# itailang/SampleNet

Hardware: NVIDIA H100
Metric: point-clouds/sec SampleNet fwd+Chamfer (B=32, N=1024->64) (higher is better)
Workload: dtype f32

## Files before the change

samplenet_b200/csrc/conv_stack.cu:

```cuda
#include "encoder_internal.cuh"
#include <cooperative_groups.h>
#include <string.h>

namespace snb {

constexpr int kCsMaxLayers = SNB200_MAX_CONV_LAYERS;
constexpr int kCsMaxSlicesPerCta = 32;
constexpr int kCsThreads = 512;
constexpr int kCsMaxPts = 128;
constexpr int kCsMinPts = 64;
constexpr int kCsNPT = kCsMaxPts / 4;
constexpr int kCsChunks = 4;
constexpr int kCsMaxSeg = 8;
constexpr int kCsLoPlane = kCsMaxPts * 128;
constexpr uint32_t kCsSlotBytes = 2u * kCsLoPlane;
constexpr int kCsWLd = 132;
constexpr uint32_t kCsWOff = kCsChunks * kCsSlotBytes;
constexpr uint32_t kCsAccOff = 2 * kCsSlotBytes;
constexpr size_t kCsSmemBytes = (size_t)kCsWOff + 128 * kCsWLd * sizeof(float) + 1024;

struct CsLayer {
    int c_in, c_out;
    const float *weight, *bias;
    const float *gamma, *beta, *run_mean, *run_var;
    float eps;
    int has_bn, relu;
    double *stats;
    float *zsave;
    int keep;
};

struct CsParams {
    const float *x; int layout;
    int b, n;
    long long total;
    int ppc, npt;
    int slots_per_cloud;
    int num_layers;
    CsLayer L[kCsMaxLayers];
    int training;
    double *mom;
    unsigned *barrier;
    float *tile_max, *tile_min;
    int fuse_head;
    HeadParams H;
    int self_clean;
    char *clean_ptr;
    unsigned clean_bytes;
    int slices_per_cta, num_slices;
    float *act[2];
    int act_ld;
    int head_rows;
};

__device__ __forceinline__ void cs_grid_arrive(unsigned *counter)
{
    asm volatile("red.release.gpu.global.add.u32 [%0], 1;" ::"l"(counter) : "memory");
}
__device__ __forceinline__ void cs_grid_wait(unsigned *counter, unsigned target)
{
    unsigned v, spin = 0;
    do {
        asm volatile("ld.acquire.gpu.global.u32 %0, [%1];" : "=r"(v) : "l"(counter) : "memory");
        if (++spin > (1u << 26)) __trap();
    } while (v < target);
}
__device__ __forceinline__ void cs_grid_barrier(unsigned *counter, unsigned target)
{
    __syncthreads();
    if (threadIdx.x == 0) {
        __threadfence();
        atomicAdd(counter, 1u);
        unsigned v, spin = 0;
        do {
            asm volatile("ld.acquire.gpu.global.u32 %0, [%1];" : "=r"(v) : "l"(counter) : "memory");
            if (++spin > (1u << 26)) __trap();
        } while (v < target);
    }
    __syncthreads();
}

__device__ __forceinline__ void cs_xchg_store(float *p, float v)
{
    unsigned u = __float_as_uint(v);
    if (u == 0u) u = 0x80000000u;
    asm volatile("st.volatile.global.u32 [%0], %1;" ::"l"(p), "r"(u) : "memory");
}
__device__ __forceinline__ unsigned cs_xchg_load1(const float *p)
{
    unsigned v;
    asm volatile("ld.volatile.global.u32 %0, [%1];" : "=r"(v) : "l"(p) : "memory");
    return v;
}
__device__ __forceinline__ uint4 cs_xchg_load4(const float *p)
{
    uint4 v;
    asm volatile("ld.volatile.global.v4.u32 {%0, %1, %2, %3}, [%4];" : "=r"(v.x), "=r"(v.y), "=r"(v.z), "=r"(v.w) : "l"(p) : "memory");
    return v;
}

__device__ __forceinline__ void cs_head_stage_weights(const HeadLayer &L, int cb, int nch, float *s_wh, int tid)
{
    const int c_in = L.c_in;
    if ((c_in & 3) == 0) {
        const int q4 = c_in >> 2, total = 8 * q4;
        for (int e0 = tid; e0 < total; e0 += kCsThreads * 4) {
            float4 v[4];
#pragma unroll
            for (int u = 0; u < 4; u++) {
                const int e = e0 + u * kCsThreads;
                const int jr = e / q4, kq = e - jr * q4;
                v[u] = (e < total && jr < nch) ? __ldg(reinterpret_cast<const float4 *>(L.weight + (size_t)(cb + jr) * c_in) + kq) : make_float4(0, 0, 0, 0);
// ... 90 lines not shown
    return v;
}
__device__ __forceinline__ void cs_named_sync(int id, int nthreads) { asm volatile("bar.sync %0, %1;" ::"r"(id), "r"(nthreads) : "memory"); }

#ifdef SNB200_CS_TIMELINE
constexpr int kCsTlMaxCtas = 256, kCsTlMaxSlices = 8;
constexpr int kCsTlPerLayer = 2 + 5 * kCsTlMaxSlices;
constexpr int kCsTlHead = 2 + (kCsMaxLayers - 1) * kCsTlPerLayer, kCsTlStamps = kCsTlHead + 2;
__device__ unsigned long long g_cs_tl[kCsTlMaxCtas][kCsTlStamps][2];
__device__ __forceinline__ int cs_tl_layer(int l) { return 2 + (l - 1) * kCsTlPerLayer; }
__device__ __forceinline__ void cs_tl_stamp(int idx)
{
    if (threadIdx.x == 0 && blockIdx.x < kCsTlMaxCtas && idx >= 0 && idx < kCsTlStamps) {
        unsigned long long c, t;
        asm volatile("mov.u64 %0, %%clock64;" : "=l"(c) :: "memory");
        asm volatile("mov.u64 %0, %%globaltimer;" : "=l"(t) :: "memory");
        g_cs_tl[blockIdx.x][idx][0] = c;
        g_cs_tl[blockIdx.x][idx][1] = t;
    }
}
#define CS_TL(idx) cs_tl_stamp(idx)
#define CS_TL_SLICE(l, t, k) do { if ((t) < kCsTlMaxSlices) cs_tl_stamp(cs_tl_layer(l) + 1 + 5 * (t) + (k)); } while (0)
#else
#define CS_TL(idx) do { } while (0)
#define CS_TL_SLICE(l, t, k) do { } while (0)
#endif

__device__ __forceinline__ void cs_copy_w(float *sW, const CsLayer &L, int ch, int g, uint64_t *bar)
{
    const int K = L.c_in, N = L.c_out;
    if (ch < N) {
        if (g == 0) {
            fence_proxy_async();
            if (ch == 0) mbar_expect_tx(bar, (uint32_t)(N * K) * 4u);
            tma_load_1d(sW + (size_t)ch * kCsWLd, L.weight + (size_t)ch * K, (uint32_t)K * 4u, bar);
        }
    } else {
        float4 *z = reinterpret_cast<float4 *>(sW + (size_t)ch * kCsWLd + g * (K >> 2));
#pragma unroll
        for (int i = 0; i < 8; i++)
            if (i * 16 < K) z[i] = make_float4(0.f, 0.f, 0.f, 0.f);
    }
}
__device__ __forceinline__ void cs_wait_w(uint64_t *bar, int c) { mbar_wait(bar, (uint32_t)c & 1u); }

__device__ __forceinline__ void cs_wg_wait_1() { asm volatile("wgmma.wait_group.sync.aligned 1;" ::: "memory"); }

__device__ __forceinline__ void cs_write_chunk(const uint32_t (&v)[kCsNPT], float sc, float sh, float floor_v, int npt, uint32_t base, uint32_t gsw)
{
#pragma unroll
    for (int jb = 0; jb < kCsNPT / 8; jb++) {
        if (jb * 8 < npt) {
#pragma unroll
            for (int i = 0; i < 8; i++) {
                const float t = fmaxf(fmaf(__uint_as_float(v[jb * 8 + i]), sc, sh), floor_v);
                const float h = tf32_hi(t);
                const uint32_t a = base + (gsw ^ (uint32_t)(i << 4)) + (uint32_t)(jb * 1024 + i * 128);
                asm volatile("st.shared.f32 [%0], %1;" ::"r"(a), "f"(h) : "memory");
                asm volatile("st.shared.f32 [%0], %1;" ::"r"(a + (uint32_t)kCsLoPlane), "f"(t - h) : "memory");
            }
        }
    }
}

__device__ __forceinline__ int cs_acc_idx(int pt, int ch) { return pt * 128 + (ch ^ (((pt >> 1) & 3) << 3)); }

__device__ __forceinline__ void cs_save_rows(float *dst, int ld, const uint32_t (&v)[kCsNPT], int nvalid)
{
#pragma unroll
    for (int j = 0; j < kCsNPT; j++)
        if (j < nvalid) dst[j * ld] = __uint_as_float(v[j]);
}

__device__ __forceinline__ void cs_load_rows(const float *src, int ld, uint32_t (&v)[kCsNPT], int nvalid)
{
#pragma unroll
    for (int j = 0; j < kCsNPT; j++) v[j] = (j < nvalid) ? __float_as_uint(__ldcg(src + j * ld)) : 0u;
}

template <bool kMulti>
__global__ void __launch_bounds__(kCsThreads, 1) conv_stack_kernel(const __grid_constant__ CsParams P)
{
    extern __shared__ __align__(1024) unsigned char smem_raw[];
    __shared__ __align__(16) float sX[kCsMaxPts * 3];
    __shared__ float sW1[128 * 3], sB1[128];
    __shared__ float sRedS[4][128], sRedQ[4][128];
    __shared__ double sMom[9];
    __shared__ float sMomW[kCsThreads / 32][9];
    __shared__ int sBad;
    __shared__ uint64_t sWbar;

    const int tid = threadIdx.x, warp = tid >> 5, lane = tid & 31;
    const int q = warp & 3, g = (warp >> 2) & 3;
    const int ch = q * 32 + lane;
    const int G = gridDim.x;
    const int ppc = P.ppc, npt = P.npt, n = P.n;
    const long long P0 = (long long)blockIdx.x * ppc;
    const int npts = (int)min((long long)ppc, P.total - P0);
    const int col0 = g * npt;
    const int nvalid = max(0, min(npt, npts - col0));
    unsigned char *smem = smem_raw + ((1024u - (smem_u32(smem_raw) & 1023u)) & 1023u);
    float *sW = reinterpret_cast<float *>(smem + kCsWOff);
    float *sAcc = reinterpret_cast<float *>(smem + kCsAccOff);
    CS_TL(0);

    if (tid < 9) sMom[tid] = 0.0;
    if (tid == 0) sBad = 0;
    if (warp == 1) {
        if (lane == 0) mbar_init(&sWbar, 1);
        fence_mbar_init();
    }
    const CsLayer &L1 = P.L[0];
    const int nslices = kMulti ? (P.num_slices - (int)blockIdx.x + G - 1) / G : 1;
    auto load_x_slice = [&](const long long P0s, const int nptss) {
        if (P.layout == SNB200_BNC) {
            const float *src = P.x + P0s * 3;
            const int nf = nptss * 3;
            for (int e = tid; e < ppc * 3; e += kCsThreads) sX[e] = (e < nf) ? __ldg(src + e) : 0.f;
        } else {
            for (int e = tid; e < ppc * 3; e += kCsThreads) {
                const int c = e / ppc, r = e - c * ppc;
                float xv = 0.f;
                if (r < nptss) {
                    const int gp = (int)P0s + r;
                    const int cloud = gp / n, pi = gp - cloud * n;
                    xv = __ldg(P.x + ((size_t)cloud * 3 + c) * n + pi);
                }
                sX[r * 3 + c] = xv;
            }
        }
    };
    if (!kMulti) load_x_slice(P0, npts);
    for (int e = tid; e < L1.c_out * 3; e += kCsThreads) sW1[e] = __ldg(L1.weight + e);
    for (int e = tid; e < L1.c_out; e += kCsThreads) sB1[e] = L1.bias ? __ldg(L1.bias + e) : 0.f;
    __syncthreads();
    unsigned barrier_epoch = 0;
    const bool need_stats = P.training != 0;
    if (P.self_clean) {
        float4 *z = reinterpret_cast<float4 *>(P.clean_ptr);
        const unsigned n16 = P.clean_bytes >> 4;
        for (unsigned e = blockIdx.x * kCsThreads + tid; e < n16; e += G * kCsThreads) z[e] = make_float4(0.f, 0.f, 0.f, 0.f);
        if (!(need_stats && L1.has_bn)) cs_grid_barrier(P.barrier, ++barrier_epoch * G);
    }

    cs_copy_w(sW, P.L[1], ch, g, &sWbar);

    if (need_stats && L1.has_bn) {
        const int mom_pts = kMulti ? ppc : npts;
        float a9[9] = {0, 0, 0, 0, 0, 0, 0, 0, 0};
        for (int t = 0; t < nslices; t++) {
            int nptss = npts;
            if (kMulti) {
                const long long P0s = (long long)((int)blockIdx.x + t * G) * ppc;
                nptss = (int)min((long long)ppc, P.total - P0s);
                __syncthreads();
                load_x_slice(P0s, nptss);
                __syncthreads();
            }
            if (tid < nptss) {
                const float px = sX[tid * 3 + 0], py = sX[tid * 3 + 1], pz = sX[tid * 3 + 2];
                a9[0] += px; a9[1] += py; a9[2] += pz;
                a9[3] = fmaf(px, px, a9[3]); a9[4] = fmaf(px, py, a9[4]); a9[5] = fmaf(px, pz, a9[5]);
                a9[6] = fmaf(py, py, a9[6]); a9[7] = fmaf(py, pz, a9[7]); a9[8] = fmaf(pz, pz, a9[8]);
            }
        }
        if (warp * 32 < mom_pts) {
#pragma unroll
            for (int j = 0; j < 9; j++) {
                float v = a9[j];
                for (int o = 16; o > 0; o >>= 1) v += __shfl_xor_sync(kFullMask, v, o);
                if (lane == 0) sMomW[warp][j] = v;
            }
        }
        __syncthreads();
        if (tid < 9) {
            double t = 0.0;
            for (int w = 0; w * 32 < mom_pts && w < kCsThreads / 32; w++) t += (double)sMomW[w][tid];
            atomicAdd(P.mom + tid, t);
            cs_grid_arrive(reinterpret_cast<unsigned *>(P.mom + 9));
        }
    }
    if (need_stats && L1.has_bn) {
        if (tid < 9) {
            cs_grid_wait(reinterpret_cast<unsigned *>(P.mom + 9), 9u * G);
            sMom[tid] = __ldcg(P.mom + tid);
        }
        __syncthreads();
    }
    CS_TL(1);

    uint32_t v[kCsNPT];
    auto layer1_eval = [&](const long long P0s, const int nvalids) {
        if (q * 32 < L1.c_out) {
            const bool cv = ch < L1.c_out;
            const float w0 = cv ? sW1[ch * 3 + 0] : 0.f, w1 = cv ? sW1[ch * 3 + 1] : 0.f, w2 = cv ? sW1[ch * 3 + 2] : 0.f, b1 = cv ? sB1[ch] : 0.f;
#pragma unroll
            for (int jb = 0; jb < kCsNPT / 8; jb++) {
                if (jb * 8 < npt) {
                    const float4 *xq = reinterpret_cast<const float4 *>(sX + (col0 + jb * 8) * 3);
                    float xr[24];
#pragma unroll
                    for (int u = 0; u < 6; u++) { const float4 t4 = xq[u]; xr[u * 4 + 0] = t4.x; xr[u * 4 + 1] = t4.y; xr[u * 4 + 2] = t4.z; xr[u * 4 + 3] = t4.w; }
#pragma unroll
                    for (int i = 0; i < 8; i++) v[jb * 8 + i] = __float_as_uint(fmaf(w2, xr[i * 3 + 2], fmaf(w1, xr[i * 3 + 1], w0 * xr[i * 3 + 0])) + b1);
                }
            }
            if (L1.zsave && cv) cs_save_rows(L1.zsave + ((int)P0s + col0) * L1.c_out + ch, L1.c_out, v, nvalids);
        }
    };
    if (!kMulti) layer1_eval(P0, nvalid);

    for (int l = 1; l < P.num_layers; l++) {
        const CsLayer &Lp = P.L[l - 1];
        const CsLayer &Lc = P.L[l];
        const int K = Lc.c_in, N = Lc.c_out;
        const int nchunks = K >> 5;
        const bool last = (l == P.num_layers - 1);
        const bool want_stats = need_stats && Lc.has_bn;

        {
            float sc = 1.f, sh = 0.f;
            if (Lp.has_bn && ch < K && g == 0) {
                const float pgamma = cs_ld_now(Lp.gamma + ch), pbeta = cs_ld_now(Lp.beta + ch);

                float mean, var;
                if (P.training) {
                    const double cnt = (double)P.total, inv_cnt = 1.0 / cnt;
                    double m, vv;
                    if (l == 1) {
                        const double mx = sMom[0] * inv_cnt, my = sMom[1] * inv_cnt, mz = sMom[2] * inv_cnt;
                        const double cxx = sMom[3] * inv_cnt - mx * mx, cxy = sMom[4] * inv_cnt - mx * my, cxz = sMom[5] * inv_cnt - mx * mz;
                        const double cyy = sMom[6] * inv_cnt - my * my, cyz = sMom[7] * inv_cnt - my * mz, czz = sMom[8] * inv_cnt - mz * mz;
                        const double a0 = sW1[ch * 3 + 0], a1 = sW1[ch * 3 + 1], a2 = sW1[ch * 3 + 2];
                        m = a0 * mx + a1 * my + a2 * mz + (double)sB1[ch];
                        vv = a0 * a0 * cxx + a1 * a1 * cyy + a2 * a2 * czz + 2.0 * (a0 * a1 * cxy + a0 * a2 * cxz + a1 * a2 * cyz);
                        if (vv < 0) vv = 0;
                        if (blockIdx.x == 0) {
                            Lp.stats[ch] = cnt * m;
                            Lp.stats[K + ch] = cnt * (vv + m * m);
                        }
                    } else {
                        double s1, s2;
                        cs_fx_collect(Lp.stats, K, ch, (unsigned)G, s1, s2);
                        if (blockIdx.x == 0) { Lp.stats[ch] = s1; Lp.stats[K + ch] = s2; }
                        m = s1 * inv_cnt;
                        vv = s2 * inv_cnt - m * m;
                        if (vv < 0) vv = 0;
                    }
                    mean = (float)m; var = (float)vv;
                } else {
                    mean = Lp.run_mean[ch]; var = Lp.run_var[ch];
                }
                const float invstd = 1.0f / sqrtf(var + Lp.eps);
                sc = pgamma * invstd;
                sh = pbeta - mean * sc;
            }
            if (Lp.has_bn) {
                if (g == 0 && ch < K) { sRedS[0][ch] = sc; sRedQ[0][ch] = sh; }
                cs_named_sync(1, kCsThreads);
                if (ch < K) { sc = sRedS[0][ch]; sh = sRedQ[0][ch]; }
                cs_named_sync(1, kCsThreads);
            }
            CS_TL(cs_tl_layer(l));
            const int mh = g & 1, nh = g >> 1;
            const bool mma_wg = mh * 64 < N && nh * 64 < ppc;
            const float bias = (ch < N && Lc.bias) ? __ldg(Lc.bias + ch) : 0.f;
            float sumL = 0.f, sqL = 0.f;
            const float *act_in = kMulti && l > 1 ? (Lp.zsave ? Lp.zsave : P.act[(l - 1) & 1]) : nullptr;
            float *act_out = kMulti && !last ? (Lc.zsave ? Lc.zsave : P.act[l & 1]) : Lc.zsave;
            const int ld_in = (kMulti && !Lp.zsave && P.act_ld) ? P.act_ld : K, ld_out = (kMulti && !last && !Lc.zsave && P.act_ld) ? P.act_ld : N;
            auto write_tiles = [&](const int sl, const int cl_first, const int nseg, const float *sPmax, const float *sPmin) {
                const int S = P.slots_per_cloud;
                for (int e = tid; e < nseg * N; e += kCsThreads) {
                    const int s = e / N, c = e - s * N;
                    const int cl = cl_first + s;
                    const int slot = sl - cl * n / ppc;
                    float mx = -INFINITY, mn = INFINITY;
#pragma unroll
                    for (int gg = 0; gg < 4; gg++) {
                        mx = fmaxf(mx, sPmax[(gg * kCsMaxSeg + s) * 128 + c]);
                        mn = fminf(mn, sPmin[(gg * kCsMaxSeg + s) * 128 + c]);
                    }
                    if (sBad) { mx = INFINITY; mn = -INFINITY; }
                    P.tile_max[((size_t)cl * S + slot) * N + c] = mx;
                    P.tile_min[((size_t)cl * S + slot) * N + c] = mn;
                    if (((cl + 1) * n - 1) / ppc == sl)
                        for (int s2 = slot + 1; s2 < S; s2++) {
                            P.tile_max[((size_t)cl * S + s2) * N + c] = -INFINITY;
                            P.tile_min[((size_t)cl * S + s2) * N + c] = INFINITY;
                        }
                }
            };
            int cl_first = 0, nseg = 0;
            float *sPmax = reinterpret_cast<float *>(smem);
            float *sPmin = sPmax + 4 * kCsMaxSeg * 128;
            for (int t = 0; t < nslices; t++) {
                const int tv = kMulti && (l & 1) ? nslices - 1 - t : t;
                const int sl = kMulti ? (int)blockIdx.x + tv * cs_nctaid() : (int)blockIdx.x;
                const long long P0 = (long long)sl * ppc;
                const int npts = (int)min((long long)ppc, P.total - P0);
                const int nvalid = max(0, min(npt, npts - col0));
                const bool lastslice = !kMulti || t == nslices - 1;
                const bool kept = kMulti && nslices - 1 - t < Lc.keep;
                if (kMulti) {
#pragma unroll
                    for (int j = 0; j < kCsNPT; j++) v[j] = 0u;
                    const bool on_chip = t < Lp.keep;
                    if (l == 1) {
                        if (!on_chip) {
                            __syncthreads();
                            load_x_slice(P0, npts);
                            __syncthreads();
                        }
                        layer1_eval(P0, nvalid);
                    } else if (on_chip && t == 0) {
                        const float pbias = (ch < K && Lp.bias) ? __ldg(Lp.bias + ch) : 0.f;
#pragma unroll
                        for (int j = 0; j < kCsNPT; j++) v[j] = __float_as_uint(sAcc[col0 * 128 + cs_acc_idx(j, ch)] + pbias);
                        if (nchunks > 2) __syncthreads();
                    } else if (ch < K) {
                        if (on_chip) {
                            const float *src = sW + col0 * kCsWLd + 64 + ch;
#pragma unroll
                            for (int j = 0; j < kCsNPT; j++) v[j] = (j < nvalid) ? __float_as_uint(src[j * kCsWLd]) : 0u;
                        } else {
                            cs_load_rows(act_in + ((int)P0 + col0) * ld_in + ch, ld_in, v, nvalid);
                        }
                    }
                }
                CS_TL_SLICE(l, t, 0);
                if (q < nchunks) {
                    const uint32_t base = smem_u32(smem) + (uint32_t)q * kCsSlotBytes + (uint32_t)col0 * 128u + (uint32_t)((lane & 3) << 2);
                    cs_write_chunk(v, sc, sh, Lp.relu ? 0.f : -INFINITY, npt, base, (uint32_t)((lane >> 2) << 4));
                    fence_proxy_async();
                }
                if (kMulti && lastslice && t > 0 && Lc.keep >= 2 && ch < N) {
#pragma unroll
                    for (int j = 0; j < kCsNPT; j++) v[j] = __float_as_uint(sAcc[col0 * 128 + cs_acc_idx(j, ch)] + bias);
                    cs_save_rows(sW + col0 * kCsWLd + 64 + ch, kCsWLd, v, npt);
                }
                if (t == 0 && tid == 0) cs_wait_w(&sWbar, l - 1);
                __syncthreads();
                CS_TL_SLICE(l, t, 1);
                float acc[32];
                if (mma_wg) {
#pragma unroll
                    for (int i = 0; i < 32; i++) acc[i] = 0.f;
                    const float *wrow = sW + (size_t)(mh * 64 + q * 16 + (lane >> 2)) * kCsWLd + (lane & 3);
                    const uint32_t bbase = smem_u32(smem) + (uint32_t)nh * 64u * 128u;
                    uint32_t ahi[2][4], alo[2][4];
#pragma unroll 1
                    for (int c = 0; c < nchunks; c++) {
                        const uint32_t sb = bbase + (uint32_t)c * kCsSlotBytes;
#pragma unroll
                        for (int ks = 0; ks < 4; ks++) {
                            float w[4];
#pragma unroll
                            for (int e = 0; e < 4; e++) w[e] = wrow[(e & 1) * 8 * kCsWLd + c * 32 + ks * 8 + (e >> 1) * 4];
                            cs_wg_wait_1();
#pragma unroll
                            for (int e = 0; e < 4; e++) {
                                const float h = tf32_hi(w[e]);
                                ahi[ks & 1][e] = __float_as_uint(h);
                                alo[ks & 1][e] = __float_as_uint(w[e] - h);
                            }
                            wg_fence();
                            const uint64_t b_hi = wg_sdesc(sb + (uint32_t)(ks * 32));
                            const uint64_t b_lo = wg_sdesc(sb + (uint32_t)(kCsLoPlane + ks * 32));
                            wg_mma_rs_n64(acc, alo[ks & 1], b_hi, (c > 0 || ks > 0) ? 1u : 0u);
                            wg_mma_rs_n64(acc, ahi[ks & 1], b_lo, 1u);
                            wg_mma_rs_n64(acc, ahi[ks & 1], b_hi, 1u);
                            wg_commit();
                        }
                    }
                    wg_wait_all();
                }
                CS_TL_SLICE(l, t, 2);
                __syncthreads();
                if (mma_wg) {
                    const int r0 = mh * 64 + q * 16 + (lane >> 2), cq = nh * 64 + 2 * (lane & 3);
                    float *st0 = sAcc + cs_acc_idx(cq, r0), *st8 = sAcc + cs_acc_idx(cq, r0 + 8);
#pragma unroll
                    for (int j = 0; j < 8; j++) {
                        st0[j * 1024] = acc[4 * j + 0];
                        st0[j * 1024 + 128] = acc[4 * j + 1];
                        st8[j * 1024] = acc[4 * j + 2];
                        st8[j * 1024 + 128] = acc[4 * j + 3];
                    }
                }
                __syncthreads();
                if (!last && lastslice) cs_copy_w(sW, P.L[l + 1], ch, g, &sWbar);
                cl_first = (int)P0 / n;
                nseg = ((int)P0 + npts - 1) / n - cl_first + 1;
#pragma unroll
                for (int j = 0; j < kCsNPT; j++) v[j] = __float_as_uint(sAcc[col0 * 128 + cs_acc_idx(j, ch)]);
                CS_TL_SLICE(l, t, 3);
                if (q * 32 < N) {
                    float sum = 0.f, sq = 0.f;
#pragma unroll
                    for (int j = 0; j < kCsNPT; j++) {
                        const float u = __uint_as_float(v[j]) + bias;
                        v[j] = __float_as_uint(u);
                        if (j < nvalid) { sum += u; sq = fmaf(u, u, sq); }
                    }
                    if (kMulti) { sumL += sum; sqL += sq; }
                    else if (want_stats) { sRedS[g][ch] = sum; sRedQ[g][ch] = sq; }
                    if (act_out && ch < N && (Lc.zsave || !kept)) cs_save_rows(act_out + ((int)P0 + col0) * ld_out + ch, ld_out, v, nvalid);
                    if (last) {
                        for (int sgi = 0; sgi < nseg; sgi++) { sPmax[(g * kCsMaxSeg + sgi) * 128 + ch] = -INFINITY; sPmin[(g * kCsMaxSeg + sgi) * 128 + ch] = INFINITY; }
                        const long long gp0 = P0 + col0;
                        const int cl = (int)gp0 / n;
                        const int first_nb = (int)((long long)(cl + 1) * n - gp0);
                        if (nvalid == npt && first_nb >= npt) {
                            float mx = -INFINITY, mn = INFINITY;
#pragma unroll
                            for (int jb = 0; jb < kCsNPT / 8; jb++) {
                                if (jb * 8 < npt) {
#pragma unroll
                                    for (int i = 0; i < 8; i++) { mx = fmaxf(mx, __uint_as_float(v[jb * 8 + i])); mn = fminf(mn, __uint_as_float(v[jb * 8 + i])); }
                                }
                            }
                            sPmax[(g * kCsMaxSeg + cl - cl_first) * 128 + ch] = mx; sPmin[(g * kCsMaxSeg + cl - cl_first) * 128 + ch] = mn;
                        } else {
                            int jlo = 0;
                            for (int c2 = cl; jlo < nvalid; c2++) {
                                const int jhi = min(nvalid, (int)((long long)(c2 + 1) * n - gp0));
                                float mx = -INFINITY, mn = INFINITY;
#pragma unroll
                                for (int j = 0; j < kCsNPT; j++) {
                                    const bool in = j >= jlo && j < jhi;
                                    mx = in ? fmaxf(mx, __uint_as_float(v[j])) : mx;
                                    mn = in ? fminf(mn, __uint_as_float(v[j])) : mn;
                                }
                                sPmax[(g * kCsMaxSeg + c2 - cl_first) * 128 + ch] = mx; sPmin[(g * kCsMaxSeg + c2 - cl_first) * 128 + ch] = mn;
                                jlo = jhi;
                            }
                        }
                    }
                }
                if (kMulti) {
                    cs_named_sync(1, kCsThreads);
                    if (last) {
                        write_tiles(sl, cl_first, nseg, sPmax, sPmin);
                        cs_named_sync(1, kCsThreads);
                    }
                }
                CS_TL_SLICE(l, t, 4);
            }
            if (kMulti && want_stats && q * 32 < N) { sRedS[g][ch] = sumL; sRedQ[g][ch] = sqL; }
            if (want_stats || last) cs_named_sync(1, kCsThreads);
            if (want_stats && g == 0 && ch < N) {
                const float sm = (sRedS[0][ch] + sRedS[1][ch]) + (sRedS[2][ch] + sRedS[3][ch]);
                const float sqq = (sRedQ[0][ch] + sRedQ[1][ch]) + (sRedQ[2][ch] + sRedQ[3][ch]);
                if (last) {
                    double *acc = Lc.stats + 2 * N;
                    atomicAdd(acc + (size_t)ch * kStatStride, (double)sm);
                    atomicAdd(acc + (size_t)(N + ch) * kStatStride, (double)sqq);
                } else if (!cs_fx_contribute(Lc.stats, N, ch, sm, sqq)) {
                    sBad = 1;
                }
            }
            if (last && !kMulti) write_tiles((int)blockIdx.x, cl_first, nseg, sPmax, sPmin);
            if (want_stats && last) {
                cs_named_sync(1, kCsThreads);
                if (tid == 0) {
                    cs_grid_arrive(P.barrier);
                    cs_grid_wait(P.barrier, (barrier_epoch + 1) * G);
                }
                cs_named_sync(1, kCsThreads);
            } else if (!last && !want_stats) {
                cs_named_sync(1, kCsThreads);
            }
            CS_TL(cs_tl_layer(l) + kCsTlPerLayer - 1);
        }
        if (want_stats && last) barrier_epoch++;
    }

    __syncthreads();
    CS_TL(kCsTlHead);

    asm volatile("griddepcontrol.launch_dependents;" ::: "memory");
    if (!P.fuse_head) {
        const CsLayer &LL = P.L[P.num_layers - 1];
        if (blockIdx.x == 0 && need_stats && LL.has_bn && tid < 2 * LL.c_out) LL.stats[tid] = cs_stat(LL.stats, 2 * LL.c_out, tid, 1);
        CS_TL(kCsTlHead + 1);
        return;
    }
    const HeadParams &H = P.H;
    float *s_in = reinterpret_cast<float *>(smem_raw);
    int hcmax = H.c_feat, hcsum = 0;
    for (int l = 0; l < H.num_fc; l++) { hcmax = max(hcmax, H.fc[l].c_in); hcsum += H.fc[l].c_in; }
    const int RS = P.head_rows, gpb = RS >> 5;
    float *s_part = reinterpret_cast<float *>(smem_raw) + (size_t)RS * (hcmax + 1);
    float *s_wall = s_part + 8 * 8 * 32;
    __shared__ uint64_t hbar[SNB200_MAX_FC_LAYERS];
    const double inv_cnt_h = 1.0 / H.count;
    const float inv_b = 1.0f / (float)H.b;
    if (tid == 0) {
        for (int l = 0; l < H.num_fc; l++) mbar_init(&hbar[l], 1);
        fence_mbar_init();
        fence_proxy_async();
        int woff = 0;
        for (int l = 0; l < H.num_fc; l++) {
            const HeadLayer &L = H.fc[l];
            const int cpc = max(8, (((L.c_out + G - 1) / G + 7) / 8) * 8);
            const int lo = blockIdx.x * cpc, hi = min(L.c_out, lo + cpc);
            const bool tma_ok = (L.c_in & 3) == 0 && (hcmax & 3) == 0 && (reinterpret_cast<uintptr_t>(L.weight) & 15) == 0;
            if (lo < hi && tma_ok) {
                const uint32_t bytes = (uint32_t)min(8, hi - lo) * L.c_in * 4u;
                mbar_expect_tx(&hbar[l], bytes);
                tma_load_1d(s_wall + woff, L.weight + (size_t)lo * L.c_in, bytes, &hbar[l]);
            }
            woff += 8 * L.c_in;
        }
    }
    if (!(need_stats && P.L[P.num_layers - 1].has_bn)) cs_grid_barrier(P.barrier, ++barrier_epoch * G);
    {
        const int total = H.b * H.c_feat;
        const int gt = (G - 1 - (int)blockIdx.x) * kCsThreads + tid, gn = G * kCsThreads;
        float *ll0 = H.ll[0];
        for (int e = gt; e < total; e += gn) {
            const int bi = e / H.c_feat, c = e % H.c_feat;
            float mx = -INFINITY, mn = INFINITY;
            const float *tm = H.tile_max + (size_t)bi * H.tiles_per_cloud * H.c_feat + c;
            const float *tn = H.tile_min + (size_t)bi * H.tiles_per_cloud * H.c_feat + c;
            const double st0 = (H.last_has_bn && H.training) ? cs_stat(H.last_stats, 2 * H.c_feat, c, H.stat_rep) : 0.0;
            const double st1 = (H.last_has_bn && H.training) ? cs_stat(H.last_stats, 2 * H.c_feat, H.c_feat + c, H.stat_rep) : 0.0;
            if (H.stat_rep && bi == 0 && H.last_has_bn && H.training) {
                double *canon = const_cast<double *>(H.last_stats);
                canon[c] = st0; canon[H.c_feat + c] = st1;
            }
            const float lg = H.last_has_bn ? __ldg(H.last_gamma + c) : 1.f, lb = H.last_has_bn ? __ldg(H.last_beta + c) : 0.f;
            for (int t0 = 0; t0 < H.tiles_per_cloud; t0 += 8) {
                float a8[8], b8[8];
#pragma unroll
                for (int u = 0; u < 8; u++) {
// ... 246 lines not shown
                P.barrier[1] = 0u;
            }
        }
    }
    CS_TL(kCsTlHead + 1);
}

struct CsPartition { int ppc, slices, grid, per_cta; };
static CsPartition cs_partition(long long total)
{
    const int sms = num_sms();
    const long long rounds = max(1ll, (total + (long long)sms * kCsMaxPts - 1) / ((long long)sms * kCsMaxPts));
    long long ppc = (total + sms * rounds - 1) / (sms * rounds);
    ppc = (ppc + 31) / 32 * 32;
    if (ppc < kCsMinPts) ppc = kCsMinPts;
    if (ppc > kCsMaxPts) ppc = kCsMaxPts;
    CsPartition R;
    R.ppc = (int)ppc;
    R.slices = (int)((total + ppc - 1) / ppc);
    R.grid = min(sms, R.slices);
    R.per_cta = (R.slices + R.grid - 1) / R.grid;
    return R;
}
static int cs_points_per_cta(long long total) { return cs_partition(total).ppc; }

void conv_stack_partition(int b, int n, int *ppc, int *slices, int *grid, int *per_cta, int *slots)
{
    const CsPartition R = cs_partition((long long)b * n);
    *ppc = R.ppc; *slices = R.slices; *grid = R.grid; *per_cta = R.per_cta;
    *slots = (n - 1) / R.ppc + 2;
}

int conv_stack_slots_per_cloud(int b, int n)
{
    const int ppc = cs_points_per_cta((long long)b * n);
    return (n - 1) / ppc + 2;
}

bool conv_stack_supported(int b, int n, int nconv, const snb200_layer *conv)
{
    if (nconv < 2 || nconv > kCsMaxLayers || conv[0].c_in != 3) return false;
    if (conv[0].c_out % 32 != 0 || conv[0].c_out > 128) return false;
    for (int l = 1; l < nconv; l++) {
        if ((conv[l].c_in != 32 && conv[l].c_in != 64 && conv[l].c_in != 128) || conv[l].c_out > 128 || conv[l].c_out < 8) return false;
        if (reinterpret_cast<uintptr_t>(conv[l].weight) & 15) return false;
    }
    const long long total = (long long)b * n;
    const CsPartition R = cs_partition(total);
    if (R.per_cta > kCsMaxSlicesPerCta) return false;
    if ((R.ppc - 1) / n + 2 > kCsMaxSeg) return false;
    if (R.grid > 255) return false;
    return true;
}

int launch_conv_stack(int b, int n, int layout, const float *x, int nconv, const snb200_layer *conv, int training, double *const *stats,
                      double *mom, unsigned *barrier, float *tile_max, float *tile_min, const HeadParams *head,
                      char *clean_ptr, size_t clean_bytes, cudaStream_t stream, float *const *zsave, float *const *act)
{
    CsParams P;
    memset(&P, 0, sizeof(P));
    if (head) { P.fuse_head = 1; P.H = *head; }
    if (head && clean_ptr) { P.self_clean = 1; P.clean_ptr = clean_ptr; P.clean_bytes = (unsigned)clean_bytes; }
    P.x = x; P.layout = layout; P.b = b; P.n = n;
    P.total = (long long)b * n;
    const CsPartition R = cs_partition(P.total);
    P.ppc = R.ppc; P.slices_per_cta = R.per_cta; P.num_slices = R.slices;
    const bool multi = R.per_cta > 1;
    if (multi && !(act && act[0] && act[1])) { set_error("conv stack: %d slices per CTA need the activation workspace", R.per_cta); return SNB200_EINVAL; }
    if (act) { P.act[0] = act[0]; P.act[1] = act[1]; }
    bool layers_ordered = training != 0;
    for (int l = 0; l < nconv; l++) layers_ordered = layers_ordered && conv[l].bn_weight != nullptr;
    P.act_ld = 0;
    if (!layers_ordered) { P.act_ld = 8; for (int l = 0; l + 1 < nconv; l++) P.act_ld = max(P.act_ld, conv[l].c_out); }
    P.npt = P.ppc / 4;
    P.slots_per_cloud = (n - 1) / P.ppc + 2;
    P.num_layers = nconv; P.training = training;
    P.mom = mom; P.barrier = barrier; P.tile_max = tile_max; P.tile_min = tile_min;
    for (int l = 0; l < nconv; l++) {
        CsLayer &D = P.L[l];
        D.c_in = conv[l].c_in; D.c_out = conv[l].c_out; D.weight = conv[l].weight; D.bias = conv[l].bias;
        D.gamma = conv[l].bn_weight; D.beta = conv[l].bn_bias; D.run_mean = conv[l].bn_running_mean; D.run_var = conv[l].bn_running_var;
        D.eps = conv[l].bn_eps; D.has_bn = conv[l].bn_weight != nullptr; D.relu = conv[l].relu; D.stats = stats[l];
        D.zsave = zsave ? zsave[l] : nullptr;
        if (!multi || l == nconv - 1) D.keep = 0;
        else if (l == 0) D.keep = (training && D.has_bn) ? 1 : 0;
        else D.keep = (D.c_in <= 64 && D.c_out <= 64) ? 2 : 1;
    }
    if (head) {
        P.H.tiles_per_cloud = P.slots_per_cloud;
        P.H.stat_rep = 1;
        for (int i = 0; i < P.H.ru_num; i++) P.H.ru_rep[i] = (P.H.ru_stats[i] == stats[nconv - 1]) ? 1 : 0;
    }
    size_t smem = kCsSmemBytes;
    if (head) {
        int hcmax = head->c_feat;
        for (int l = 0; l < head->num_fc; l++) hcmax = max(hcmax, head->fc[l].c_in);
        size_t hcsum = 0;
        for (int l = 0; l < head->num_fc; l++) hcsum += head->fc[l].c_in;
        int rs = min(128, (b + 31) / 32 * 32);
        size_t hs = 0;
        for (;; rs -= 32) {
            hs = ((size_t)rs * (hcmax + 1) + 2048 + (size_t)8 * hcsum) * sizeof(float) + 1024;
            if (hs <= 200 * 1024 || rs == 32) break;
        }
        if (hs > 200 * 1024) { set_error("conv stack: FC width %d too large for the fused head", hcmax); return SNB200_EUNSUPPORTED; }
        P.head_rows = rs;
        smem = max(smem, hs);
    }
    static PerDeviceOnce once;
    if (once.first()) {
        cudaFuncSetAttribute(conv_stack_kernel<false>, cudaFuncAttributeMaxDynamicSharedMemorySize, 204 * 1024);
        cudaFuncSetAttribute(conv_stack_kernel<true>, cudaFuncAttributeMaxDynamicSharedMemorySize, 204 * 1024);
    }
    const int grid = R.grid;
    cudaLaunchConfig_t cfg;
    memset(&cfg, 0, sizeof(cfg));
    cfg.gridDim = dim3(grid); cfg.blockDim = dim3(kCsThreads); cfg.dynamicSmemBytes = smem; cfg.stream = stream;
    cudaLaunchAttribute attr[1];
    attr[0].id = cudaLaunchAttributeCooperative;
    attr[0].val.cooperative = 1;
    cfg.attrs = attr; cfg.numAttrs = 1;
    cudaError_t e = multi ? cudaLaunchKernelEx(&cfg, conv_stack_kernel<true>, P) : cudaLaunchKernelEx(&cfg, conv_stack_kernel<false>, P);
    if (e != cudaSuccess) { set_error("conv stack: cooperative launch failed: %s", cudaGetErrorString(e)); cudaGetLastError(); return SNB200_ECUDA; }
    return check_launch("conv stack");
}

}

#ifdef SNB200_CS_TIMELINE
extern "C" __attribute__((visibility("default"))) int snb200_cs_timeline(unsigned long long *host, size_t bytes)
{
    void *dev = nullptr;
    if (bytes != sizeof(snb::g_cs_tl) || cudaDeviceSynchronize() != cudaSuccess) return -1;
    if (cudaMemcpyFromSymbol(host, snb::g_cs_tl, bytes) != cudaSuccess || cudaGetSymbolAddress(&dev, snb::g_cs_tl) != cudaSuccess) return -1;
    if (cudaMemset(dev, 0, bytes) != cudaSuccess || cudaDeviceSynchronize() != cudaSuccess) return -1;
    return snb::kCsTlStamps;
}
extern "C" __attribute__((visibility("default"))) int snb200_cs_timeline_layout(int *max_ctas, int *max_slices, int *per_layer, int *head)
{
    *max_ctas = snb::kCsTlMaxCtas; *max_slices = snb::kCsTlMaxSlices; *per_layer = snb::kCsTlPerLayer; *head = snb::kCsTlHead;
    return snb::kCsTlStamps;
}
#endif
```

Before: 280,600.

## Pair two point slices per pass for narrow conv layers in multi-slice mode

For middle conv layers with at most 64 input and output channels, the multi-slice kernel now handles two point slices per pass. Each half of the channel warps and each pair of warpgroups works on its own slice, so the 128-wide MMA tile is filled instead of half of it idling. This halves the number of passes, barriers and weight waits for those layers, and lets two slices stay on chip between layers. In exchange it adds double-buffered input slices and considerably more intricate indexing for on-chip reuse and stats reduction, which risks correctness problems. It only takes effect when more than one slice is assigned per CTA.

```diff
diff --git a/samplenet_b200/csrc/conv_stack.cu b/samplenet_b200/csrc/conv_stack.cu
--- a/samplenet_b200/csrc/conv_stack.cu
+++ b/samplenet_b200/csrc/conv_stack.cu
@@ -28,6 +28,7 @@
     double *stats;
     float *zsave;
     int keep;
+    int pair;
 };
 
 struct CsParams {
@@ -284,7 +285,7 @@
 __global__ void __launch_bounds__(kCsThreads, 1) conv_stack_kernel(const __grid_constant__ CsParams P)
 {
     extern __shared__ __align__(1024) unsigned char smem_raw[];
-    __shared__ __align__(16) float sX[kCsMaxPts * 3];
+    __shared__ __align__(16) float sX[kMulti ? 2 : 1][kCsMaxPts * 3];
     __shared__ float sW1[128 * 3], sB1[128];
     __shared__ float sRedS[4][128], sRedQ[4][128];
     __shared__ double sMom[9];
@@ -314,11 +315,11 @@
     }
     const CsLayer &L1 = P.L[0];
     const int nslices = kMulti ? (P.num_slices - (int)blockIdx.x + G - 1) / G : 1;
-    auto load_x_slice = [&](const long long P0s, const int nptss) {
+    auto load_x_slice = [&](const long long P0s, const int nptss, float *xs) {
         if (P.layout == SNB200_BNC) {
             const float *src = P.x + P0s * 3;
             const int nf = nptss * 3;
-            for (int e = tid; e < ppc * 3; e += kCsThreads) sX[e] = (e < nf) ? __ldg(src + e) : 0.f;
+            for (int e = tid; e < ppc * 3; e += kCsThreads) xs[e] = (e < nf) ? __ldg(src + e) : 0.f;
         } else {
             for (int e = tid; e < ppc * 3; e += kCsThreads) {
                 const int c = e / ppc, r = e - c * ppc;
@@ -328,11 +329,12 @@
                     const int cloud = gp / n, pi = gp - cloud * n;
                     xv = __ldg(P.x + ((size_t)cloud * 3 + c) * n + pi);
                 }
-                sX[r * 3 + c] = xv;
+                xs[r * 3 + c] = xv;
             }
         }
     };
-    if (!kMulti) load_x_slice(P0, npts);
+    auto slice_p0 = [&](const int tv) { return (long long)((int)blockIdx.x + tv * cs_nctaid()) * ppc; };
+    if (!kMulti) load_x_slice(P0, npts, sX[0]);
     for (int e = tid; e < L1.c_out * 3; e += kCsThreads) sW1[e] = __ldg(L1.weight + e);
     for (int e = tid; e < L1.c_out; e += kCsThreads) sB1[e] = L1.bias ? __ldg(L1.bias + e) : 0.f;
     __syncthreads();
@@ -353,14 +355,15 @@
         for (int t = 0; t < nslices; t++) {
             int nptss = npts;
             if (kMulti) {
-                const long long P0s = (long long)((int)blockIdx.x + t * G) * ppc;
+                const long long P0s = slice_p0(t);
                 nptss = (int)min((long long)ppc, P.total - P0s);
                 __syncthreads();
-                load_x_slice(P0s, nptss);
+                load_x_slice(P0s, nptss, sX[t & 1]);
                 __syncthreads();
             }
             if (tid < nptss) {
-                const float px = sX[tid * 3 + 0], py = sX[tid * 3 + 1], pz = sX[tid * 3 + 2];
+                const float *xs = sX[kMulti ? t & 1 : 0];
+                const float px = xs[tid * 3 + 0], py = xs[tid * 3 + 1], pz = xs[tid * 3 + 2];
                 a9[0] += px; a9[1] += py; a9[2] += pz;
                 a9[3] = fmaf(px, px, a9[3]); a9[4] = fmaf(px, py, a9[4]); a9[5] = fmaf(px, pz, a9[5]);
                 a9[6] = fmaf(py, py, a9[6]); a9[7] = fmaf(py, pz, a9[7]); a9[8] = fmaf(pz, pz, a9[8]);
@@ -392,14 +395,14 @@
     CS_TL(1);
 
     uint32_t v[kCsNPT];
-    auto layer1_eval = [&](const long long P0s, const int nvalids) {
-        if (q * 32 < L1.c_out) {
-            const bool cv = ch < L1.c_out;
-            const float w0 = cv ? sW1[ch * 3 + 0] : 0.f, w1 = cv ? sW1[ch * 3 + 1] : 0.f, w2 = cv ? sW1[ch * 3 + 2] : 0.f, b1 = cv ? sB1[ch] : 0.f;
+    auto layer1_eval = [&](const long long P0s, const int nvalids, const float *xs, const int c) {
+        if ((c & ~31) < L1.c_out) {
+            const bool cv = c < L1.c_out;
+            const float w0 = cv ? sW1[c * 3 + 0] : 0.f, w1 = cv ? sW1[c * 3 + 1] : 0.f, w2 = cv ? sW1[c * 3 + 2] : 0.f, b1 = cv ? sB1[c] : 0.f;
 #pragma unroll
             for (int jb = 0; jb < kCsNPT / 8; jb++) {
                 if (jb * 8 < npt) {
-                    const float4 *xq = reinterpret_cast<const float4 *>(sX + (col0 + jb * 8) * 3);
+                    const float4 *xq = reinterpret_cast<const float4 *>(xs + (col0 + jb * 8) * 3);
                     float xr[24];
 #pragma unroll
                     for (int u = 0; u < 6; u++) { const float4 t4 = xq[u]; xr[u * 4 + 0] = t4.x; xr[u * 4 + 1] = t4.y; xr[u * 4 + 2] = t4.z; xr[u * 4 + 3] = t4.w; }
@@ -407,10 +410,10 @@
                     for (int i = 0; i < 8; i++) v[jb * 8 + i] = __float_as_uint(fmaf(w2, xr[i * 3 + 2], fmaf(w1, xr[i * 3 + 1], w0 * xr[i * 3 + 0])) + b1);
                 }
             }
-            if (L1.zsave && cv) cs_save_rows(L1.zsave + ((int)P0s + col0) * L1.c_out + ch, L1.c_out, v, nvalids);
+            if (L1.zsave && cv) cs_save_rows(L1.zsave + ((int)P0s + col0) * L1.c_out + c, L1.c_out, v, nvalids);
         }
     };
-    if (!kMulti) layer1_eval(P0, nvalid);
+    if (!kMulti) layer1_eval(P0, nvalid, sX[0], ch);
 
     for (int l = 1; l < P.num_layers; l++) {
         const CsLayer &Lp = P.L[l - 1];
@@ -419,6 +422,9 @@
         const int nchunks = K >> 5;
         const bool last = (l == P.num_layers - 1);
         const bool want_stats = need_stats && Lc.has_bn;
+        const bool pair = kMulti && Lc.pair;
+        const int mem = pair ? q >> 1 : 0;
+        const int c = pair ? ch & 63 : ch;
 
         {
             float sc = 1.f, sh = 0.f;
@@ -460,13 +466,12 @@
             if (Lp.has_bn) {
                 if (g == 0 && ch < K) { sRedS[0][ch] = sc; sRedQ[0][ch] = sh; }
                 cs_named_sync(1, kCsThreads);
-                if (ch < K) { sc = sRedS[0][ch]; sh = sRedQ[0][ch]; }
+                if (c < K) { sc = sRedS[0][c]; sh = sRedQ[0][c]; }
                 cs_named_sync(1, kCsThreads);
             }
             CS_TL(cs_tl_layer(l));
             const int mh = g & 1, nh = g >> 1;
-            const bool mma_wg = mh * 64 < N && nh * 64 < ppc;
-            const float bias = (ch < N && Lc.bias) ? __ldg(Lc.bias + ch) : 0.f;
+            const float bias = (c < N && Lc.bias) ? __ldg(Lc.bias + c) : 0.f;
             float sumL = 0.f, sqL = 0.f;
             const float *act_in = kMulti && l > 1 ? (Lp.zsave ? Lp.zsave : P.act[(l - 1) & 1]) : nullptr;
             float *act_out = kMulti && !last ? (Lc.zsave ? Lc.zsave : P.act[l & 1]) : Lc.zsave;
@@ -496,69 +501,96 @@
             int cl_first = 0, nseg = 0;
             float *sPmax = reinterpret_cast<float *>(smem);
             float *sPmin = sPmax + 4 * kCsMaxSeg * 128;
-            for (int t = 0; t < nslices; t++) {
-                const int tv = kMulti && (l & 1) ? nslices - 1 - t : t;
-                const int sl = kMulti ? (int)blockIdx.x + tv * cs_nctaid() : (int)blockIdx.x;
-                const long long P0 = (long long)sl * ppc;
-                const int npts = (int)min((long long)ppc, P.total - P0);
-                const int nvalid = max(0, min(npt, npts - col0));
-                const bool lastslice = !kMulti || t == nslices - 1;
-                const bool kept = kMulti && nslices - 1 - t < Lc.keep;
+            const bool fwd = !(kMulti && (l & 1));
+            const int e_in = (l & 1) ? nslices - 1 : 0;
+            auto on_chip = [&](const int s) { return Lp.keep > 0 && (Lp.pair ? (s >> 1) == (e_in >> 1) : s == e_in); };
+            for (int t = 0, pass = 0; t < nslices; pass++) {
+                const int us = !pair ? 1 : fwd ? min(2, nslices - t) : 2 - ((nslices - t) & 1);
+                const int tv0 = fwd ? t : nslices - t - us;
+                const bool has_slice = mem < us;
+                auto geometry = [&](const int m, int &P0, int &npts, int &nvalid) {
+                    P0 = (kMulti ? (int)blockIdx.x + (tv0 + m) * cs_nctaid() : (int)blockIdx.x) * ppc;
+                    npts = (int)min((long long)ppc, P.total - P0);
+                    nvalid = max(0, min(npt, npts - col0));
+                };
+                const bool lastslice = !kMulti || t + us == nslices;
+                const bool kept = kMulti && Lc.keep > 0 && lastslice;
                 if (kMulti) {
 #pragma unroll
                     for (int j = 0; j < kCsNPT; j++) v[j] = 0u;
-                    const bool on_chip = t < Lp.keep;
                     if (l == 1) {
-                        if (!on_chip) {
+                        if (!on_chip(tv0)) {
                             __syncthreads();
-                            load_x_slice(P0, npts);
+#pragma unroll 1
+                            for (int m = 0; m < us; m++) {
+                                const long long P0m = slice_p0(tv0 + m);
+                                load_x_slice(P0m, (int)min((long long)ppc, P.total - P0m), sX[(tv0 + m) & 1]);
+                            }
                             __syncthreads();
                         }
-                        layer1_eval(P0, nvalid);
-                    } else if (on_chip && t == 0) {
-                        const float pbias = (ch < K && Lp.bias) ? __ldg(Lp.bias + ch) : 0.f;
-#pragma unroll
-                        for (int j = 0; j < kCsNPT; j++) v[j] = __float_as_uint(sAcc[col0 * 128 + cs_acc_idx(j, ch)] + pbias);
-                        if (nchunks > 2) __syncthreads();
-                    } else if (ch < K) {
-                        if (on_chip) {
-                            const float *src = sW + col0 * kCsWLd + 64 + ch;
+                    }
+#pragma unroll 1
+                    for (int m = 0; m < us; m++) {
+                        if (m != mem) continue;
+                        const int tv = tv0 + m;
+                        int P0, npts, nvalid;
+                        geometry(m, P0, npts, nvalid);
+                        if (l == 1) {
+                            layer1_eval(P0, nvalid, sX[tv & 1], c);
+                            continue;
+                        }
+                        if (c >= K) continue;
+                        const bool oc = on_chip(tv);
+                        if (oc && (pair || t == 0)) {
+                            const int h = Lp.pair ? tv & 1 : 0;
+                            const float pbias = Lp.bias ? __ldg(Lp.bias + c) : 0.f;
+#pragma unroll
+                            for (int j = 0; j < kCsNPT; j++) v[j] = __float_as_uint(sAcc[col0 * 128 + cs_acc_idx(j, h * 64 + c)] + pbias);
+                        } else if (oc) {
+                            const float *src = sW + col0 * kCsWLd + 64 + c;
 #pragma unroll
                             for (int j = 0; j < kCsNPT; j++) v[j] = (j < nvalid) ? __float_as_uint(src[j * kCsWLd]) : 0u;
                         } else {
-                            cs_load_rows(act_in + ((int)P0 + col0) * ld_in + ch, ld_in, v, nvalid);
-                        }
-                    }
-                }
-                CS_TL_SLICE(l, t, 0);
-                if (q < nchunks) {
+                            cs_load_rows(act_in + (P0 + col0) * ld_in + c, ld_in, v, nvalid);
+                        }
+                    }
+                    if (l > 1 && !pair && t == 0 && Lp.pair && q >= 2 && ch - 64 < K) {
+                        const int tn = fwd ? tv0 + 1 : tv0 - 1;
+                        if (nslices > 1 && on_chip(tn)) {
+                            const int cp = ch - 64;
+                            const float pbias = Lp.bias ? __ldg(Lp.bias + cp) : 0.f;
+#pragma unroll
+                            for (int j = 0; j < kCsNPT; j++) v[j] = __float_as_uint(sAcc[col0 * 128 + cs_acc_idx(j, (tn & 1) * 64 + cp)] + pbias);
+                            cs_save_rows(sW + col0 * kCsWLd + 64 + cp, kCsWLd, v, npt);
+                        }
+                    }
+                    if (l > 1 && t == 0 && Lp.keep > 0 && (pair || nchunks > 2)) __syncthreads();
+                }
+                CS_TL_SLICE(l, pass, 0);
+                if (pair ? has_slice && (q & 1) < nchunks : q < nchunks) {
                     const uint32_t base = smem_u32(smem) + (uint32_t)q * kCsSlotBytes + (uint32_t)col0 * 128u + (uint32_t)((lane & 3) << 2);
                     cs_write_chunk(v, sc, sh, Lp.relu ? 0.f : -INFINITY, npt, base, (uint32_t)((lane >> 2) << 4));
                     fence_proxy_async();
                 }
-                if (kMulti && lastslice && t > 0 && Lc.keep >= 2 && ch < N) {
-#pragma unroll
-                    for (int j = 0; j < kCsNPT; j++) v[j] = __float_as_uint(sAcc[col0 * 128 + cs_acc_idx(j, ch)] + bias);
-                    cs_save_rows(sW + col0 * kCsWLd + 64 + ch, kCsWLd, v, npt);
-                }
                 if (t == 0 && tid == 0) cs_wait_w(&sWbar, l - 1);
                 __syncthreads();
-                CS_TL_SLICE(l, t, 1);
+                CS_TL_SLICE(l, pass, 1);
                 float acc[32];
+                const bool mma_wg = (pair || mh * 64 < N) && nh * 64 < ppc;
                 if (mma_wg) {
 #pragma unroll
                     for (int i = 0; i < 32; i++) acc[i] = 0.f;
-                    const float *wrow = sW + (size_t)(mh * 64 + q * 16 + (lane >> 2)) * kCsWLd + (lane & 3);
-                    const uint32_t bbase = smem_u32(smem) + (uint32_t)nh * 64u * 128u;
+                    const float *wrow = sW + (size_t)((pair ? 0 : mh * 64) + q * 16 + (lane >> 2)) * kCsWLd + (lane & 3);
+                    const uint32_t bbase = smem_u32(smem) + (pair ? (uint32_t)mh * 2u * kCsSlotBytes : 0u) + (uint32_t)nh * 64u * 128u;
                     uint32_t ahi[2][4], alo[2][4];
 #pragma unroll 1
-                    for (int c = 0; c < nchunks; c++) {
-                        const uint32_t sb = bbase + (uint32_t)c * kCsSlotBytes;
+                    for (int kc = 0; kc < nchunks; kc++) {
+                        const uint32_t sb = bbase + (uint32_t)kc * kCsSlotBytes;
 #pragma unroll
                         for (int ks = 0; ks < 4; ks++) {
                             float w[4];
 #pragma unroll
-                            for (int e = 0; e < 4; e++) w[e] = wrow[(e & 1) * 8 * kCsWLd + c * 32 + ks * 8 + (e >> 1) * 4];
+                            for (int e = 0; e < 4; e++) w[e] = wrow[(e & 1) * 8 * kCsWLd + kc * 32 + ks * 8 + (e >> 1) * 4];
                             cs_wg_wait_1();
 #pragma unroll
                             for (int e = 0; e < 4; e++) {
@@ -569,7 +601,7 @@
                             wg_fence();
                             const uint64_t b_hi = wg_sdesc(sb + (uint32_t)(ks * 32));
                             const uint64_t b_lo = wg_sdesc(sb + (uint32_t)(kCsLoPlane + ks * 32));
-                            wg_mma_rs_n64(acc, alo[ks & 1], b_hi, (c > 0 || ks > 0) ? 1u : 0u);
+                            wg_mma_rs_n64(acc, alo[ks & 1], b_hi, (kc > 0 || ks > 0) ? 1u : 0u);
                             wg_mma_rs_n64(acc, ahi[ks & 1], b_lo, 1u);
                             wg_mma_rs_n64(acc, ahi[ks & 1], b_hi, 1u);
                             wg_commit();
@@ -577,7 +609,7 @@
                     }
                     wg_wait_all();
                 }
-                CS_TL_SLICE(l, t, 2);
+                CS_TL_SLICE(l, pass, 2);
                 __syncthreads();
                 if (mma_wg) {
                     const int r0 = mh * 64 + q * 16 + (lane >> 2), cq = nh * 64 + 2 * (lane & 3);
@@ -592,50 +624,56 @@
                 }
                 __syncthreads();
                 if (!last && lastslice) cs_copy_w(sW, P.L[l + 1], ch, g, &sWbar);
-                cl_first = (int)P0 / n;
-                nseg = ((int)P0 + npts - 1) / n - cl_first + 1;
 #pragma unroll
                 for (int j = 0; j < kCsNPT; j++) v[j] = __float_as_uint(sAcc[col0 * 128 + cs_acc_idx(j, ch)]);
-                CS_TL_SLICE(l, t, 3);
-                if (q * 32 < N) {
-                    float sum = 0.f, sq = 0.f;
-#pragma unroll
-                    for (int j = 0; j < kCsNPT; j++) {
-                        const float u = __uint_as_float(v[j]) + bias;
-                        v[j] = __float_as_uint(u);
-                        if (j < nvalid) { sum += u; sq = fmaf(u, u, sq); }
-                    }
-                    if (kMulti) { sumL += sum; sqL += sq; }
-                    else if (want_stats) { sRedS[g][ch] = sum; sRedQ[g][ch] = sq; }
-                    if (act_out && ch < N && (Lc.zsave || !kept)) cs_save_rows(act_out + ((int)P0 + col0) * ld_out + ch, ld_out, v, nvalid);
-                    if (last) {
-                        for (int sgi = 0; sgi < nseg; sgi++) { sPmax[(g * kCsMaxSeg + sgi) * 128 + ch] = -INFINITY; sPmin[(g * kCsMaxSeg + sgi) * 128 + ch] = INFINITY; }
-                        const long long gp0 = P0 + col0;
-                        const int cl = (int)gp0 / n;
-                        const int first_nb = (int)((long long)(cl + 1) * n - gp0);
-                        if (nvalid == npt && first_nb >= npt) {
-                            float mx = -INFINITY, mn = INFINITY;
-#pragma unroll
-                            for (int jb = 0; jb < kCsNPT / 8; jb++) {
-                                if (jb * 8 < npt) {
-#pragma unroll
-                                    for (int i = 0; i < 8; i++) { mx = fmaxf(mx, __uint_as_float(v[jb * 8 + i])); mn = fminf(mn, __uint_as_float(v[jb * 8 + i])); }
+                CS_TL_SLICE(l, pass, 3);
+#pragma unroll 1
+                for (int m = 0; m < us; m++) {
+                    if (m != mem) continue;
+                    int P0, npts, nvalid;
+                    geometry(m, P0, npts, nvalid);
+                    cl_first = P0 / n;
+                    nseg = (P0 + npts - 1) / n - cl_first + 1;
+                    if ((c & ~31) < N) {
+                        float sum = 0.f, sq = 0.f;
+#pragma unroll
+                        for (int j = 0; j < kCsNPT; j++) {
+                            const float u = __uint_as_float(v[j]) + bias;
+                            v[j] = __float_as_uint(u);
+                            if (j < nvalid) { sum += u; sq = fmaf(u, u, sq); }
+                        }
+                        if (kMulti) { sumL += sum; sqL += sq; }
+                        else if (want_stats) { sRedS[g][ch] = sum; sRedQ[g][ch] = sq; }
+                        if (act_out && c < N && (Lc.zsave || !kept)) cs_save_rows(act_out + (P0 + col0) * ld_out + c, ld_out, v, nvalid);
+                        if (last) {
+                            for (int sgi = 0; sgi < nseg; sgi++) { sPmax[(g * kCsMaxSeg + sgi) * 128 + ch] = -INFINITY; sPmin[(g * kCsMaxSeg + sgi) * 128 + ch] = INFINITY; }
+                            const long long gp0 = P0 + col0;
+                            const int cl = (int)gp0 / n;
+                            const int first_nb = (int)((long long)(cl + 1) * n - gp0);
+                            if (nvalid == npt && first_nb >= npt) {
+                                float mx = -INFINITY, mn = INFINITY;
+#pragma unroll
+                                for (int jb = 0; jb < kCsNPT / 8; jb++) {
+                                    if (jb * 8 < npt) {
+#pragma unroll
+                                        for (int i = 0; i < 8; i++) { mx = fmaxf(mx, __uint_as_float(v[jb * 8 + i])); mn = fminf(mn, __uint_as_float(v[jb * 8 + i])); }
+                                    }
                                 }
-                            }
-                            sPmax[(g * kCsMaxSeg + cl - cl_first) * 128 + ch] = mx; sPmin[(g * kCsMaxSeg + cl - cl_first) * 128 + ch] = mn;
-                        } else {
-                            int jlo = 0;
-                            for (int c2 = cl; jlo < nvalid; c2++) {
-                                const int jhi = min(nvalid, (int)((long long)(c2 + 1) * n - gp0));
-                                float mx = -INFINITY, mn = INFINITY;
-#pragma unroll
-                                for (int j = 0; j < kCsNPT; j++) {
-                                    const bool in = j >= jlo && j < jhi;
-                                    mx = in ? fmaxf(mx, __uint_as_float(v[j])) : mx;
-                                    mn = in ? fminf(mn, __uint_as_float(v[j])) : mn;
+                                sPmax[(g * kCsMaxSeg + cl - cl_first) * 128 + ch] = mx; sPmin[(g * kCsMaxSeg + cl - cl_first) * 128 + ch] = mn;
+                            } else {
+                                int jlo = 0;
+                                for (int c2 = cl; jlo < nvalid; c2++) {
+                                    const int jhi = min(nvalid, (int)((long long)(c2 + 1) * n - gp0));
+                                    float mx = -INFINITY, mn = INFINITY;
+#pragma unroll
+                                    for (int j = 0; j < kCsNPT; j++) {
+                                        const bool in = j >= jlo && j < jhi;
+                                        mx = in ? fmaxf(mx, __uint_as_float(v[j])) : mx;
+                                        mn = in ? fminf(mn, __uint_as_float(v[j])) : mn;
+                                    }
+                                    sPmax[(g * kCsMaxSeg + c2 - cl_first) * 128 + ch] = mx; sPmin[(g * kCsMaxSeg + c2 - cl_first) * 128 + ch] = mn;
+                                    jlo = jhi;
                                 }
-                                sPmax[(g * kCsMaxSeg + c2 - cl_first) * 128 + ch] = mx; sPmin[(g * kCsMaxSeg + c2 - cl_first) * 128 + ch] = mn;
-                                jlo = jhi;
                             }
                         }
                     }
@@ -643,17 +681,22 @@
                 if (kMulti) {
                     cs_named_sync(1, kCsThreads);
                     if (last) {
-                        write_tiles(sl, cl_first, nseg, sPmax, sPmin);
+                        write_tiles((int)blockIdx.x + tv0 * cs_nctaid(), cl_first, nseg, sPmax, sPmin);
                         cs_named_sync(1, kCsThreads);
                     }
                 }
-                CS_TL_SLICE(l, t, 4);
-            }
-            if (kMulti && want_stats && q * 32 < N) { sRedS[g][ch] = sumL; sRedQ[g][ch] = sqL; }
+                CS_TL_SLICE(l, pass, 4);
+                t += us;
+            }
+            if (kMulti && want_stats && (c & ~31) < N) { sRedS[g][ch] = sumL; sRedQ[g][ch] = sqL; }
             if (want_stats || last) cs_named_sync(1, kCsThreads);
             if (want_stats && g == 0 && ch < N) {
-                const float sm = (sRedS[0][ch] + sRedS[1][ch]) + (sRedS[2][ch] + sRedS[3][ch]);
-                const float sqq = (sRedQ[0][ch] + sRedQ[1][ch]) + (sRedQ[2][ch] + sRedQ[3][ch]);
+                float sm = (sRedS[0][ch] + sRedS[1][ch]) + (sRedS[2][ch] + sRedS[3][ch]);
+                float sqq = (sRedQ[0][ch] + sRedQ[1][ch]) + (sRedQ[2][ch] + sRedQ[3][ch]);
+                if (pair) {
+                    sm += (sRedS[0][ch + 64] + sRedS[1][ch + 64]) + (sRedS[2][ch + 64] + sRedS[3][ch + 64]);
+                    sqq += (sRedQ[0][ch + 64] + sRedQ[1][ch + 64]) + (sRedQ[2][ch + 64] + sRedQ[3][ch + 64]);
+                }
                 if (last) {
                     double *acc = Lc.stats + 2 * N;
                     atomicAdd(acc + (size_t)ch * kStatStride, (double)sm);
@@ -1066,9 +1109,14 @@
         D.gamma = conv[l].bn_weight; D.beta = conv[l].bn_bias; D.run_mean = conv[l].bn_running_mean; D.run_var = conv[l].bn_running_var;
         D.eps = conv[l].bn_eps; D.has_bn = conv[l].bn_weight != nullptr; D.relu = conv[l].relu; D.stats = stats[l];
         D.zsave = zsave ? zsave[l] : nullptr;
+        D.pair = multi && l > 0 && l < nconv - 1 && D.c_in <= 64 && D.c_out <= 64;
+    }
+    P.L[0].pair = P.L[1].pair;
+    for (int l = 0; l < nconv; l++) {
+        CsLayer &D = P.L[l];
         if (!multi || l == nconv - 1) D.keep = 0;
-        else if (l == 0) D.keep = (training && D.has_bn) ? 1 : 0;
-        else D.keep = (D.c_in <= 64 && D.c_out <= 64) ? 2 : 1;
+        else if (l == 0) D.keep = (training && D.has_bn) ? (D.pair ? 2 : 1) : 0;
+        else D.keep = D.pair ? 2 : 1;
     }
     if (head) {
         P.H.tiles_per_cloud = P.slots_per_cloud;
```

New measurement: 292,900 (median of 6 runs). 1.04x the previous value.
